# TJUMMG/OCPG

Hardware: AMD Instinct MI355X
Metric: clips/sec fwd+bwd (5x384x640, R101) (higher is better)
Workload: dtype bf16

## Files before the change

### include/ocpg_hip.h

```cpp
#ifndef OCPG_HIP_H
#define OCPG_HIP_H
#include <stdint.h>

#ifdef __cplusplus
extern "C" {
#endif

int ocpg_msda_fwd_f32(const float* value, const int64_t* shapes, const int64_t* level_start,
                      const float* loc, const float* attn,
                      int N, int S, int M, int D, int L, int Lq, int P,
                      float* out, const int64_t* shapes_host, void* stream);
int ocpg_msda_fwd_f64(const double* value, const int64_t* shapes, const int64_t* level_start,
                      const double* loc, const double* attn,
                      int N, int S, int M, int D, int L, int Lq, int P,
                      double* out, void* stream);

int ocpg_msda_bwd_f32(const float* value, const int64_t* shapes, const int64_t* level_start,
                      const float* loc, const float* attn, const float* grad_out,
                      int N, int S, int M, int D, int L, int Lq, int P,
                      float* grad_value, float* grad_loc, float* grad_attn,
                      const int64_t* shapes_host, void* stream);
int ocpg_msda_bwd_value_f32(const float* loc, const float* attn, const float* grad_out,
                            int N, int S, int M, int D, int L, int Lq, int P,
                            float* grad_value, const int64_t* shapes_host, void* stream);
// ... 11 lines not shown
                                  float* grad_qproj, void* stream);
int ocpg_msda_bwd_value_sel_f32(const float* loc, const float* attn, const float* grad_out,
                                int N, int S, int M, int D, int L, int Lq, int P,
                                float* grad_value, const int64_t* shapes_host, int* sel_state, void* stream);
int ocpg_msda_bwd_f64(const double* value, const int64_t* shapes, const int64_t* level_start,
                      const double* loc, const double* attn, const double* grad_out,
                      int N, int S, int M, int D, int L, int Lq, int P,
                      double* grad_value, double* grad_loc, double* grad_attn, void* stream);

int ocpg_msda_sf_fwd_f32(const float* src, const float* wv, const float* bv, const unsigned char* pad,
                         const int64_t* shapes, const int64_t* level_start, const float* loc, const float* attn,
                         int N, int S, int M, int D, int L, int Lq, int P,
                         float* out, float* s, float* beta, void* stream);
int ocpg_msda_sf_bwd_f32(const float* src, const float* wv, const float* bv, const unsigned char* pad,
                         const int64_t* shapes, const int64_t* level_start, const float* loc, const float* attn,
                         const float* grad_out, int N, int S, int M, int D, int L, int Lq, int P,
                         float* grad_src, float* grad_loc, float* grad_attn, void* stream);
int ocpg_msda_sf_bwd_params_f32(const float* grad_out, const float* s, const float* beta, int N, int M, int D, int Lq,
                                float* grad_wv, float* grad_bv, void* stream);

int ocpg_msda_fwd_h16(const void* value, const int64_t* shapes, const int64_t* level_start,
                      const float* loc, const float* attn,
                      int N, int S, int M, int D, int L, int Lq, int P,
                      void* out, const int64_t* shapes_host, int dtype, void* stream);
int ocpg_msda_bwd_h16(const void* value, const int64_t* shapes, const int64_t* level_start,
                      const float* loc, const float* attn, const void* grad_out,
                      int N, int S, int M, int D, int L, int Lq, int P,
                      float* grad_value, float* grad_loc, float* grad_attn,
                      const int64_t* shapes_host, int* sel_state, int dtype, void* stream);
int ocpg_msda_bwd_value_h16(const float* loc, const float* attn, const void* grad_out,
                            int N, int S, int M, int D, int L, int Lq, int P,
                            float* grad_value, const int64_t* shapes_host, int* sel_state, int dtype, void* stream);
int ocpg_msda_bwd_locattn_h16(const void* value, const int64_t* shapes, const int64_t* level_start,
                              const float* loc, const float* attn, const void* grad_out,
                              int N, int S, int M, int D, int L, int Lq, int P,
                              float* grad_loc, float* grad_attn, int dtype, void* stream);
int ocpg_msda_fused_fwd_h16(const void* value, const int64_t* shapes, const int64_t* level_start,
                            const float* qproj, const float* ref,
                            int N, int S, int M, int D, int L, int Lq, int P,
                            void* out, float* loc_out, float* attn_out, int dtype, void* stream);
int ocpg_msda_fused_bwd_qproj_h16(const void* value, const int64_t* shapes, const int64_t* level_start,
                                  const float* loc, const float* attn, const void* grad_out,
                                  int N, int S, int M, int D, int L, int Lq, int P,
                                  float* grad_qproj, int dtype, void* stream);

int ocpg_bn_act_fwd(const void* x, const float* scale, const float* shift, const void* skip, void* y,
                    long long n_outer, int C, long long inner, int relu, int dtype, void* stream);
int ocpg_bn_act_bwd(const void* gy, const void* y, const float* scale, void* gx, void* gskip,
                    long long n_outer, int C, long long inner, int relu, int dtype, void* stream);

int ocpg_gemm_dgrad_bn_tile(long long M, int N, int K);
int ocpg_gemm_dgrad_bn(const void* a, const void* w, const void* c, const void* mask, const float* scale, void* out, void* out_skip,
                       long long M, int N, int K, int dtype, int tile, void* stream);

int ocpg_win_attn_fwd(const void* qkv, const float* biasT, const int* region, float scale, int BW, int NW, int N, int H,
                      int head_dim, void* out, float* lse, int dtype, void* stream);
int ocpg_win_attn_bwd(const void* qkv, const float* bias, const float* biasT, const int* region, float scale, int BW, int NW,
                      int N, int H, int head_dim, const void* out, const void* dout, const float* lse, void* dqkv, float* Dbuf,
                      float* dbiasT, int dtype, void* stream);

int ocpg_win_attn_bwd_mfma(const void* qkv, const float* bias, const float* biasT, const int* region, float scale, int BW, int NW, int N,
                           int H, int head_dim, const void* out, const void* dout, const float* lse, void* dqkv, float* Dbuf, void* dS,
                           int dtype, void* stream);

int ocpg_win_attn_dtable_supported(int N, int head_dim, int dtype, int T);
int ocpg_win_attn_bwd_mfma_dtable(const void* qkv, const float* bias, const float* biasT, const int* region, float scale, int BW, int NW,
                                  int N, int H, int head_dim, const void* out, const void* dout, const float* lse, void* dqkv, float* Dbuf,
                                  const int* tok_code, int code_off, int T, float* partials, float* dtable, int dtype, void* stream);

int ocpg_dynmask_fwd_f32(const float* feats, const float* params, const float* refpix, int BT, int Q, int C, int H, int W,
                         int stride, float* out, float* pre1, void* stream);

int ocpg_dynmask_bwd_pre_f32(const float* dout, const float* pre1, const float* params, int BT, int Q, int C, int H, int W,
                             int stride, float* dpre, float* part, float* w0d, void* stream);
int ocpg_dynmask_bwd_fin_f32(const float* part, const float* params, const float* refpix, const float* dw0, int BT, int Q, int C,
                             int H, int W, float* dparams, float* dref, void* stream);

int ocpg_im2col3x3_nhwc(const void* x, int N, int H, int W, int C, int stride, int dil, void* cols, int dtype, void* stream);
int ocpg_col2im3x3_nhwc(const void* dcols, int N, int H, int W, int C, int stride, int dil, void* dx, int dtype, void* stream);

int ocpg_conv3x3_mfma_fwd(const void* x, const void* w, const float* scale, const float* bias, int relu, int N, int H, int W,
                          int Cin, int Cout, int stride, void* y, void* stream);
int ocpg_conv3x3_mfma_fwd_cols(const void* x, const void* w, const float* scale, const float* bias, int relu, int N, int H, int W, int Cin,
                               int Cout, int stride, void* y, void* cols, void* stream);
int ocpg_conv3x3_mfma_dgrad(const void* dy, const void* wT, int N, int H, int W, int Cin, int Cout, int stride, void* dx,
                            void* stream);
int ocpg_conv3x3_mfma_dgrad_masked(const void* dy, const void* wT, const void* mask_y, const float* scale, int N, int H, int W, int Cin,
                                   int Cout, int stride, void* dx, void* stream);
int ocpg_conv3x3_mfma_dgrad_w(const void* dy, const void* w, const void* mask_y, const float* scale, int N, int H, int W, int Cin, int Cout,
                              int stride, void* dx, void* stream);
int ocpg_conv3x3_mfma_body_splits(long long M, int ncols, int kchannels);
int ocpg_conv3x3_mfma_fwd_bn_splitk(const void* x, const void* w, const float* scale, const float* shift, int relu, int N, int H, int W, int Cin,
                                    int Cout, int stride, int splits, float* part, void* y, void* stream);
int ocpg_conv3x3_mfma_dgrad_w_splitk(const void* dy, const void* w, const void* mask_y, const float* scale, int N, int H, int W, int Cin,
                                     int Cout, int stride, int splits, float* part, void* dx, void* stream);
int ocpg_conv3x3_mfma_wgrad_splits(int N, int H, int W, int Cin, int Cout, int stride);
int ocpg_conv3x3_mfma_wgrad(const void* gz, const void* x, int N, int H, int W, int Cin, int Cout, int stride, void* part, void* stream);
int ocpg_conv3x3_mfma_fwd_cols_h16(const void* x, const void* w, const float* scale, const float* bias, int relu, int N, int H, int W, int Cin,
                                   int Cout, int stride, void* y, void* cols, int dtype, void* stream);
int ocpg_conv3x3_mfma_dgrad_w_h16(const void* dy, const void* w, const void* mask_y, const float* scale, int N, int H, int W, int Cin, int Cout,
                                  int stride, void* dx, int dtype, void* stream);
int ocpg_conv3x3_mfma_wgrad_h16(const void* gz, const void* x, int N, int H, int W, int Cin, int Cout, int stride, void* part, int dtype,
                                void* stream);
int ocpg_conv3x3_mfma_dgrad_w_s2(const void* dy, const void* w, const void* mask_y, const float* scale, int N, int H, int W, int Cin, int Cout,
                                 int stride, void* dx, void* stream);
int ocpg_conv3x3_mfma_dgrad_w_s2_h16(const void* dy, const void* w, const void* mask_y, const float* scale, int N, int H, int W, int Cin, int Cout,
// ... 201 lines not shown
```

### ocpg_amd/_lib.py

```python
import ctypes
import os

import torch

_HERE = os.path.dirname(os.path.abspath(__file__))
LIB_PATH = os.environ.get("OCPG_HIP_LIB") or os.path.join(_HERE, "lib", "libocpg_hip.so")
_lib = None

_i64p = ctypes.c_void_p
_vp = ctypes.c_void_p
_int = ctypes.c_int

SIGNATURES = {
    "ocpg_msda_fwd_f32": [_vp, _i64p, _i64p, _vp, _vp] + [_int] * 7 + [_vp, _vp, _vp],
    "ocpg_msda_fwd_f64": [_vp, _i64p, _i64p, _vp, _vp] + [_int] * 7 + [_vp, _vp],
    "ocpg_msda_bwd_f32": [_vp, _i64p, _i64p, _vp, _vp, _vp] + [_int] * 7 + [_vp, _vp, _vp, _vp, _vp],
    "ocpg_msda_bwd_value_f32": [_vp, _vp, _vp] + [_int] * 7 + [_vp, _vp, _vp],
    "ocpg_msda_fused_fwd_f32": [_vp, _i64p, _i64p, _vp, _vp] + [_int] * 7 + [_vp, _vp, _vp, _vp],
    "ocpg_msda_fused_bwd_qproj_f32": [_vp, _i64p, _i64p, _vp, _vp, _vp] + [_int] * 7 + [_vp, _vp],
    "ocpg_msda_bwd_value_sel_f32": [_vp, _vp, _vp] + [_int] * 7 + [_vp, _vp, _vp, _vp],
    "ocpg_msda_bwd_locattn_f32": [_vp, _i64p, _i64p, _vp, _vp, _vp] + [_int] * 7 + [_vp, _vp, _vp],
    "ocpg_msda_bwd_f64": [_vp, _i64p, _i64p, _vp, _vp, _vp] + [_int] * 7 + [_vp, _vp, _vp, _vp],
    "ocpg_msda_sf_fwd_f32": [_vp, _vp, _vp, _vp, _i64p, _i64p, _vp, _vp] + [_int] * 7 + [_vp, _vp, _vp, _vp],
    "ocpg_msda_sf_bwd_f32": [_vp, _vp, _vp, _vp, _i64p, _i64p, _vp, _vp, _vp] + [_int] * 7 + [_vp, _vp, _vp, _vp],
    "ocpg_msda_sf_bwd_params_f32": [_vp, _vp, _vp] + [_int] * 4 + [_vp, _vp, _vp],
    "ocpg_msda_fwd_h16": [_vp, _i64p, _i64p, _vp, _vp] + [_int] * 7 + [_vp, _vp, _int, _vp],
    "ocpg_msda_bwd_h16": [_vp, _i64p, _i64p, _vp, _vp, _vp] + [_int] * 7 + [_vp, _vp, _vp, _vp, _vp, _int, _vp],
    "ocpg_msda_bwd_value_h16": [_vp, _vp, _vp] + [_int] * 7 + [_vp, _vp, _vp, _int, _vp],
    "ocpg_msda_bwd_locattn_h16": [_vp, _i64p, _i64p, _vp, _vp, _vp] + [_int] * 7 + [_vp, _vp, _int, _vp],
    "ocpg_msda_fused_fwd_h16": [_vp, _i64p, _i64p, _vp, _vp] + [_int] * 7 + [_vp, _vp, _vp, _int, _vp],
    "ocpg_msda_fused_bwd_qproj_h16": [_vp, _i64p, _i64p, _vp, _vp, _vp] + [_int] * 7 + [_vp, _int, _vp],
    "ocpg_bn_act_fwd": [_vp, _vp, _vp, _vp, _vp, ctypes.c_longlong, _int, ctypes.c_longlong, _int, _int, _vp],
    "ocpg_bn_act_bwd": [_vp, _vp, _vp, _vp, _vp, ctypes.c_longlong, _int, ctypes.c_longlong, _int, _int, _vp],
    "ocpg_gemm_dgrad_bn_tile": [ctypes.c_longlong, _int, _int],
    "ocpg_gemm_dgrad_bn": [_vp] * 7 + [ctypes.c_longlong, _int, _int, _int, _int, _vp],
    "ocpg_dynmask_fwd_f32": [_vp, _vp, _vp] + [_int] * 6 + [_vp, _vp, _vp],
    "ocpg_dynmask_bwd_pre_f32": [_vp, _vp, _vp] + [_int] * 6 + [_vp, _vp, _vp, _vp],
    "ocpg_dynmask_bwd_fin_f32": [_vp, _vp, _vp, _vp] + [_int] * 5 + [_vp, _vp, _vp],
    "ocpg_conv3x3_mfma_fwd": [_vp, _vp, _vp, _vp] + [_int] * 7 + [_vp, _vp],
    "ocpg_conv3x3_mfma_fwd_cols": [_vp, _vp, _vp, _vp] + [_int] * 7 + [_vp, _vp, _vp],
    "ocpg_conv3x3_mfma_dgrad": [_vp, _vp] + [_int] * 6 + [_vp, _vp],
    "ocpg_conv3x3_mfma_dgrad_masked": [_vp, _vp, _vp, _vp] + [_int] * 6 + [_vp, _vp],
    "ocpg_conv3x3_mfma_dgrad_w": [_vp, _vp, _vp, _vp] + [_int] * 6 + [_vp, _vp],
    "ocpg_conv3x3_mfma_splits": [_int] * 6,
    "ocpg_conv3x3_mfma_wgrad_splits": [_int] * 6,
    "ocpg_conv3x3_mfma_body_splits": [ctypes.c_longlong, _int, _int],
    "ocpg_conv3x3_mfma_fwd_bn_splitk": [_vp, _vp, _vp, _vp] + [_int] * 8 + [_vp, _vp, _vp],
    "ocpg_conv3x3_mfma_dgrad_w_splitk": [_vp, _vp, _vp, _vp] + [_int] * 7 + [_vp, _vp, _vp],
    "ocpg_conv3x3_mfma_wgrad": [_vp, _vp] + [_int] * 6 + [_vp, _vp],
    "ocpg_conv3x3_mfma_fwd_cols_h16": [_vp, _vp, _vp, _vp] + [_int] * 7 + [_vp, _vp, _int, _vp],
    "ocpg_conv3x3_mfma_dgrad_w_h16": [_vp, _vp, _vp, _vp] + [_int] * 6 + [_vp, _int, _vp],
    "ocpg_conv3x3_mfma_wgrad_h16": [_vp, _vp] + [_int] * 6 + [_vp, _int, _vp],
    "ocpg_conv3x3_mfma_dgrad_w_s2": [_vp, _vp, _vp, _vp] + [_int] * 6 + [_vp, _vp],
    "ocpg_conv3x3_mfma_dgrad_w_s2_h16": [_vp, _vp, _vp, _vp] + [_int] * 6 + [_vp, _int, _vp],
    "ocpg_conv3x3_mfma_fwd_splitk": [_vp, _vp, _vp] + [_int] * 7 + [_vp, _vp, _int, _vp, _vp],
    "ocpg_conv3x3_mfma_fwd_splitk_h16": [_vp, _vp, _vp] + [_int] * 7 + [_vp, _vp, _int, _vp, _int, _vp],
    "ocpg_gemm": [_vp, _vp, _vp, _vp] + [_int] * 4 + [ctypes.c_longlong] * 10 + [ctypes.c_float, ctypes.c_float, _vp],
    "ocpg_gemm_plans": [],
    "ocpg_gemm_tuned": [_vp],
    "ocpg_gemm_tune_rejected": [],
    "ocpg_gemm_set_tuning": [_int],
    "ocpg_gemm_export_picks": [_vp, ctypes.c_longlong],
    "ocpg_gemm_import_picks": [_vp, ctypes.c_longlong],
    "ocpg_window_means3x3_fwd": [_vp, ctypes.c_longlong, _int, _int, _int, _vp, _vp],
    "ocpg_window_means3x3_bwd": [_vp, ctypes.c_longlong, _int, _int, _vp, _vp],
    "ocpg_window_sums3x3_cl_bands": [_int],
    "ocpg_window_sums3x3_cl": [_vp, _int, _int, _int, _int, _int, _vp, _vp],
    "ocpg_window_means3x3_bwd_cl": [_vp, _int, _int, _int, _int, _vp, _vp, _vp],
    "ocpg_mso_conv3x3": [_vp, _int, _int, _vp, _int, _vp, _vp, _int, _vp, _int, _vp, _vp, _int] + [_int] * 6 + [_vp],
    "ocpg_mso_wgrad_rows": [_int] * 4,
    "ocpg_mso_wgrad": [_vp, _int, _int, _vp, _vp, _vp] + [_int] * 8 + [_vp],
    "ocpg_bilinear_nhwc_fwd": [_vp] + [_int] * 6 + [_vp, _vp],
    "ocpg_bilinear_nhwc_bwd": [_vp] + [_int] * 6 + [_vp, _vp],
    "ocpg_small_linear_fwd": [_vp, _int, _vp, _vp, _int, _int, _int, _int, _vp, _vp],
    "ocpg_small_linear_bwd": [_vp, _int, _vp, _int, _vp, _vp, _int, _int, _int, _vp, _vp, _vp, _vp],
    "ocpg_small_linear_fwd_h16": [_vp, _int, _vp, _vp, _int, _int, _int, _int, _vp, _int, _vp],
    "ocpg_small_linear_bwd_h16": [_vp, _int, _vp, _int, _vp, _vp, _int, _int, _int, _vp, _vp, _vp, _int, _vp],
    "ocpg_small_linear_f32_fwd": [_vp, _vp, _vp, _int, _int, _int, _vp, _vp],
    "ocpg_small_linear_f32_bwd": [_vp, _vp, _vp, _int, _int, _int, _vp, _vp, _vp, _vp],
    "ocpg_layernorm_blocks": [ctypes.c_longlong],
    "ocpg_groupnorm_cl_work": [ctypes.c_longlong, _int, _int, _int],
    "ocpg_groupnorm_cl_fwd": [_vp, _int, _vp, _vp, ctypes.c_longlong, _int, _int, _int, ctypes.c_float, _vp, _vp, _vp, _vp, _vp],
    "ocpg_groupnorm_cl_bwd": [_vp, _vp, _int, _vp, _vp, _vp, ctypes.c_longlong, _int, _int, _int, _vp, _vp, _vp, _vp],
    "ocpg_groupnorm_cl2cl_fwd": [_vp, _int, _vp, _vp, ctypes.c_longlong, _int, _int, _int, ctypes.c_float, _vp, _vp, _vp, _vp, _vp],
    "ocpg_groupnorm_cl2cl_bwd": [_vp, _vp, _int, _vp, _vp, _vp, ctypes.c_longlong, _int, _int, _int, _vp, _vp, _vp, _vp],
    "ocpg_layernorm_fwd": [_vp, _int, _vp, _vp, ctypes.c_longlong, _int, ctypes.c_float, _vp, _int, _vp, _vp, _vp],
    "ocpg_layernorm_bwd": [_vp, _int, _vp, _int, _vp, _vp, _vp, ctypes.c_longlong, _int, _vp, _int, _vp, _vp, _vp],
    "ocpg_gather_rows_bwd": [_vp, _vp, _vp, _int, _int, _vp, _vp],
# ... 49 lines not shown
                                                             _vp, _vp, _int, _vp],
    "ocpg_attn_longk_fwd": [_vp, ctypes.c_longlong, _vp, ctypes.c_longlong, _vp, ctypes.c_longlong, _vp, ctypes.c_float] + [_int] * 5
                           + [ctypes.c_float, ctypes.c_ulonglong, ctypes.c_ulonglong, _vp, _vp, ctypes.c_longlong, _vp, _int, _vp],
    "ocpg_attn_longk_bwd": [_vp, ctypes.c_longlong, _vp, ctypes.c_longlong, _vp, ctypes.c_longlong, _vp, _vp, ctypes.c_longlong, _vp,
                            ctypes.c_longlong, _vp, ctypes.c_float] + [_int] * 5 + [ctypes.c_float, ctypes.c_ulonglong, ctypes.c_ulonglong, _vp,
                                                                                    _vp, ctypes.c_longlong, _vp, _vp, _int, _vp],
    "ocpg_text_gate_rows": [_int],
    "ocpg_text_gate_splits": [_int],
    "ocpg_text_gate_fwd_h16": [_vp] * 6 + [ctypes.c_float] + [_int] * 5 + [_vp, _int, _vp],
    "ocpg_text_gate_bwd_h16": [_vp] * 7 + [ctypes.c_float] + [_int] * 5 + [_vp, _vp, _vp, _int, _vp],
    "ocpg_mask_tail_f32": [_vp] + [_int] * 10 + [ctypes.c_float, ctypes.c_float, _int, _vp, _vp],
    "ocpg_jf_counts_u8": [_vp, _vp] + [_int] * 8 + [_vp, _vp],
    "ocpg_refmask_counts_f32": [_vp] + [_int] * 5 + [_vp] * 4 + [_int, _int, ctypes.c_float, _int, _vp, _vp],
    "ocpg_sim_heat_workspace": [_int] * 4,
    "ocpg_sim_heat_f32": [_vp] + [_int] * 5 + [_vp] * 10,
    "ocpg_win_attn_fwd": [_vp, _vp, _vp, ctypes.c_float] + [_int] * 5 + [_vp, _vp, _int, _vp],
    "ocpg_win_attn_bwd": [_vp, _vp, _vp, _vp, ctypes.c_float] + [_int] * 5 + [_vp] * 6 + [_int, _vp],
    "ocpg_win_attn_bwd_mfma": [_vp, _vp, _vp, _vp, ctypes.c_float] + [_int] * 5 + [_vp] * 6 + [_int, _vp],
    "ocpg_win_attn_dtable_supported": [_int] * 4,
    "ocpg_win_attn_bwd_mfma_dtable": [_vp, _vp, _vp, _vp, ctypes.c_float] + [_int] * 5 + [_vp] * 6 + [_int, _int, _vp, _vp, _int, _vp],
}


_TIMING = {"on": False, "events": []}
_UNTIMED = ("ocpg_sim_heat_workspace", "ocpg_text_gate_rows", "ocpg_text_gate_splits", "ocpg_win_attn_dtable_supported", "ocpg_conv3x3_mfma_body_splits", "ocpg_gemm_dgrad_bn_tile", "ocpg_conv3x3_mfma_wgrad_splits", "ocpg_window_sums3x3_cl_bands", "ocpg_lfm_dft_supported", "ocpg_lfm_dft_split", "ocpg_conv3x3_mfma_splits", "ocpg_gemm_set_tuning", "ocpg_gemm_export_picks", "ocpg_gemm_import_picks", "ocpg_colsum_blocks", "ocpg_mso_wgrad_rows", "ocpg_gemm_plans", "ocpg_gemm_tuned", "ocpg_gemm_tune_rejected", "ocpg_bias_relu_dropout_bwd_slots", "ocpg_dropout_add_ln_bwd_slots", "ocpg_groupnorm_cl_work")


def enable_kernel_timing(on=True):
    _TIMING["on"] = on
    _TIMING["events"] = []


def collect_kernel_timing(work=None):
    torch.cuda.synchronize()
    out = {}
    for name, args, e0, e1 in _TIMING["events"]:
        d = out.setdefault(name, {"ms": 0.0, "n": 0, "work": 0.0, "modelled": 0})
        d["ms"] += e0.elapsed_time(e1)
        d["n"] += 1
        w = work(name, args) if work is not None else None
        if isinstance(w, tuple):
            d["work_lowp"] = d.get("work_lowp", 0.0) + (w[0] if w[1] else 0.0)
            w = w[0]
        if w is not None:
            d["work"] += w
            d["modelled"] += 1
    _TIMING["events"] = []
    _TIMING["on"] = False
    return out


CENSUS = {"on": False, "calls": {}}
CENSUS_ALSO = {"ocpg_conv3x3_mfma_dgrad_w_s2": "ocpg_conv3x3_mfma_dgrad_w", "ocpg_conv3x3_mfma_dgrad_w_s2_h16": "ocpg_conv3x3_mfma_dgrad_w_h16",
               "ocpg_dropout_add_ln_fwd_ex": "ocpg_dropout_add_ln_fwd", "ocpg_dropout_add_ln_bwd_ex": "ocpg_dropout_add_ln_bwd"}


def census(on=True):
    CENSUS["on"] = on
    if on:
        CENSUS["calls"] = {}
    return CENSUS["calls"]


class _Lib:

    def __init__(self, cdll):
        self._cdll = cdll

    def __getattr__(self, name):
        fn = getattr(self._cdll, name)
        if name not in SIGNATURES or name in _UNTIMED:
            setattr(self, name, fn)
            return fn
        timed = not name.startswith("ocpg_msda_")

        def call(*a):
            if CENSUS["on"]:
                rc = fn(*a)
                if rc == 0:
                    for k in (name, CENSUS_ALSO.get(name)):
                        if k is not None:
                            CENSUS["calls"][k] = CENSUS["calls"].get(k, 0) + 1
                return rc
            if not (timed and _TIMING["on"]):
                return fn(*a)
            e0, e1 = torch.cuda.Event(enable_timing=True), torch.cuda.Event(enable_timing=True)
            e0.record()
            rc = fn(*a)
            e1.record()
            _TIMING["events"].append((name, tuple(getattr(x, "value", x) for x in a), e0, e1))
            return rc
        setattr(self, name, call)
        return call


def lib():
    global _lib
    if _lib is None:
        if not os.path.exists(LIB_PATH):
            raise RuntimeError(
                f"{LIB_PATH} not found: build it with `python -m ocpg_amd.csrc.build` "
                "(hipcc --offload-arch=gfx950). The HIP extension is mandatory; there is no CPU/PyTorch fallback.")
        L = ctypes.CDLL(LIB_PATH)
        for name, argtypes in SIGNATURES.items():
            fn = getattr(L, name)
            fn.argtypes = argtypes
            fn.restype = ctypes.c_int
# ... 32 lines not shown
```

### ocpg_amd/csrc/gemm_dgrad_bn.hip

```cpp
#include <hip/hip_bf16.h>
#include <hip/hip_fp16.h>
#include <hip/hip_runtime.h>
#include <stdint.h>

#include "../../include/ocpg_hip.h"
#include "h16_elem.h"

namespace {

typedef ocpg_h16::h16x8 bf16x8;
typedef short s4 __attribute__((ext_vector_type(4)));
typedef ocpg_h16::f32x16 f32x16;
typedef unsigned u32x4 __attribute__((ext_vector_type(4)));

constexpr int BK = 64, NT = 256;
constexpr int ALD = BK + 8;

constexpr int DECLINE_SHAPE = -2000, DECLINE_ALIGN = -2001, DECLINE_DTYPE = -2002;

struct Bf16 : ocpg_h16::Bf16 {
  static __device__ __forceinline__ void unpack8(const uint4 u, float (&f)[8]) {
    const uint32_t w[4] = {u.x, u.y, u.z, u.w};
#pragma unroll
    for (int i = 0; i < 4; ++i) {
// ... 15 lines not shown
#pragma unroll
    for (int i = 0; i < 4; ++i) {
      const float2 t = __half22float2(h[i]);
      f[2 * i] = t.x;
      f[2 * i + 1] = t.y;
    }
  }
  static __device__ __forceinline__ uint4 pack8(const float (&f)[8]) {
    uint32_t w[4];
#pragma unroll
    for (int i = 0; i < 4; ++i)
      w[i] = (uint32_t)__half_as_ushort(__float2half_rn(f[2 * i])) | ((uint32_t)__half_as_ushort(__float2half_rn(f[2 * i + 1])) << 16);
    return make_uint4(w[0], w[1], w[2], w[3]);
  }
};

template <typename T>
struct EpiT {
  const T* c;
  const T* mask;
  const float* scale;
  T* out;
  T* out_skip;
};
using Epi = EpiT<__hip_bfloat16>;

struct In8 { uint4 c, y; };
template <typename T>
__device__ __forceinline__ In8 load8(const EpiT<T>& e, long long off) {
  In8 r{make_uint4(0u, 0u, 0u, 0u), make_uint4(0u, 0u, 0u, 0u)};
  if (e.c) r.c = *reinterpret_cast<const uint4*>(e.c + off);
  if (e.mask) r.y = *reinterpret_cast<const uint4*>(e.mask + off);
  return r;
}

template <typename E>
__device__ __forceinline__ void epilogue8(const EpiT<typename E::T>& e, long long off, int col, float (&v)[8], const In8& in) {
  if (e.c) {
    float c[8];
    E::unpack8(in.c, c);
#pragma unroll
    for (int i = 0; i < 8; ++i) v[i] += c[i];
  }
  if (e.mask) {
    float y[8];
    E::unpack8(in.y, y);
#pragma unroll
    for (int i = 0; i < 8; ++i) v[i] = y[i] > 0.f ? v[i] : 0.f;
  }
  if (e.out_skip) *reinterpret_cast<uint4*>(e.out_skip + off) = E::pack8(v);
  if (e.scale) {
    const float4 s0 = reinterpret_cast<const float4*>(e.scale + col)[0], s1 = reinterpret_cast<const float4*>(e.scale + col)[1];
    v[0] *= s0.x, v[1] *= s0.y, v[2] *= s0.z, v[3] *= s0.w, v[4] *= s1.x, v[5] *= s1.y, v[6] *= s1.z, v[7] *= s1.w;
  }
  *reinterpret_cast<uint4*>(e.out + off) = E::pack8(v);
}

template <typename E, int TM, int TN>
__device__ __forceinline__ void gemm_dgrad_bn_body(const typename E::T* __restrict__ a, const typename E::T* __restrict__ w,
                                                   const EpiT<typename E::T>& e, long long M, int N, int K, int mtiles, int ntiles) {
  using T = typename E::T;
  constexpr int BLD = TN + 8;
  constexpr int SLD = TN + 4;
  constexpr int WM = TM / 2, WN = TN / 2, IM = WM / 32, JN = WN / 32;
  constexpr int A_L = TM * BK / 8 / NT;
  constexpr int BSEG = TN / 8, BROWS = NT / BSEG, B_L = BK / BROWS;
  constexpr int SMEM_SHORTS = 2 * (TM * ALD + BK * BLD);
  static_assert(TM * SLD * 2 <= SMEM_SHORTS, "the fp32 tile fits the staging buffers");
  __shared__ __attribute__((aligned(16))) short smem[SMEM_SHORTS];
  short (*As)[TM * ALD] = reinterpret_cast<short (*)[TM * ALD]>(smem);
  short (*Bs)[BK * BLD] = reinterpret_cast<short (*)[BK * BLD]>(smem + 2 * TM * ALD);
  const int tid = threadIdx.x, lane = tid & 63, wave = tid >> 6;
  const int wm = wave & 1, wn = wave >> 1;
  const unsigned total = gridDim.x;
  unsigned t = blockIdx.x;
  if ((total & 7u) == 0) t = (t & 7u) * (total >> 3) + (t >> 3);
  const long long m0 = (long long)(t / ntiles) * TM;
  const int n0 = (int)(t % ntiles) * TN;
  const int ksteps = K / BK;

  const int arow = tid >> 3, aseg = tid & 7, kr = tid / BSEG, bseg = tid % BSEG;
  const T* ap[A_L];
#pragma unroll
  for (int i = 0; i < A_L; ++i) {
    const long long r = min(m0 + arow + 32 * i, M - 1);
    ap[i] = a + r * K + aseg * 8;
  }
  const T* wp = w + (long long)kr * N + n0 + bseg * 8;
  const long long wstep = (long long)BROWS * N;

  auto fetch = [&](u32x4 (&Ra)[A_L], u32x4 (&Rb)[B_L], int s) __attribute__((always_inline)) {
    const int ks = min(s, ksteps - 1);
#pragma unroll
    for (int i = 0; i < A_L; ++i) Ra[i] = *reinterpret_cast<const u32x4*>(ap[i] + ks * BK);
    const T* wk = wp + (long long)ks * BK * N;
#pragma unroll
    for (int i = 0; i < B_L; ++i) Rb[i] = *reinterpret_cast<const u32x4*>(wk + i * wstep);
  };
  auto park = [&](int buf, const u32x4 (&Ra)[A_L], const u32x4 (&Rb)[B_L]) __attribute__((always_inline)) {
#pragma unroll
    for (int i = 0; i < A_L; ++i) *reinterpret_cast<u32x4*>(&As[buf][(arow + 32 * i) * ALD + aseg * 8]) = Ra[i];
#pragma unroll
    for (int i = 0; i < B_L; ++i) *reinterpret_cast<u32x4*>(&Bs[buf][(kr + BROWS * i) * BLD + bseg * 8]) = Rb[i];
  };

  f32x16 acc[IM * JN];
// ... 33 lines not shown
  park(0, R0a, R0b);
  __syncthreads();
  for (int s = 0; s < ksteps; s += 2) {
    fetch(R0a, R0b, s + 2);
    compute(0);
    park(1, R1a, R1b);
    __syncthreads();
    fetch(R1a, R1b, s + 3);
    compute(1);
    park(0, R0a, R0b);
    __syncthreads();
  }

  float* st = reinterpret_cast<float*>(smem);
  float* st0 = st + (wm * WM + 4 * fh) * SLD + wn * WN + fr;
#pragma unroll
  for (int r = 0; r < 16; ++r) {
    float* p = st0 + ((r & 3) + 8 * (r >> 2)) * SLD;
#pragma unroll
    for (int i = 0; i < IM; ++i)
#pragma unroll
      for (int j = 0; j < JN; ++j) p[i * 32 * SLD + j * 32] = acc[i * JN + j][r];
  }
  __syncthreads();
  constexpr int NQ = TM * TN / 8 / NT;
  In8 in[NQ];
#pragma unroll
  for (int q = 0; q < NQ; ++q) {
    const int idx = tid + q * NT;
    const long long grow = m0 + idx / BSEG;
    in[q] = grow < M ? load8(e, grow * N + n0 + (idx % BSEG) * 8) : In8{make_uint4(0u, 0u, 0u, 0u), make_uint4(0u, 0u, 0u, 0u)};
  }
#pragma unroll
  for (int q = 0; q < NQ; ++q) {
    const int idx = tid + q * NT, row = idx / BSEG, c8 = (idx % BSEG) * 8;
    const long long grow = m0 + row;
    if (grow >= M) continue;
    const float4 x0 = *reinterpret_cast<const float4*>(&st[row * SLD + c8]), x1 = *reinterpret_cast<const float4*>(&st[row * SLD + c8 + 4]);
    float v[8] = {x0.x, x0.y, x0.z, x0.w, x1.x, x1.y, x1.z, x1.w};
    epilogue8<E>(e, grow * N + n0 + c8, n0 + c8, v, in[q]);
  }
}

template <int TM, int TN>
__global__ __launch_bounds__(NT) void gemm_dgrad_bn(const __hip_bfloat16* __restrict__ a, const __hip_bfloat16* __restrict__ w, Epi e,
                                                    long long M, int N, int K, int mtiles, int ntiles) {
  gemm_dgrad_bn_body<Bf16, TM, TN>(a, w, e, M, N, K, mtiles, ntiles);
}

template <int TM, int TN>
__global__ __launch_bounds__(NT) void gemm_dgrad_bn_f16(const __half* __restrict__ a, const __half* __restrict__ w, EpiT<__half> e,
                                                        long long M, int N, int K, int mtiles, int ntiles) {
  gemm_dgrad_bn_body<Fp16, TM, TN>(a, w, e, M, N, K, mtiles, ntiles);
}

constexpr int TILE_M[3] = {128, 64, 64}, TILE_N[3] = {128, 128, 64};

inline bool aligned16(const void* p) { return ((uintptr_t)p & 15u) == 0; }

}

extern "C" int ocpg_gemm_dgrad_bn_tile(long long M, int N, int K) {
  if (M <= 0 || N <= 0 || K <= 0 || N % TILE_N[2] != 0 || K % (2 * BK) != 0) return -1;
  return 2;
}

extern "C" int ocpg_gemm_dgrad_bn(const void* a, const void* w, const void* c, const void* mask, const float* scale, void* out, void* out_skip,
                                  long long M, int N, int K, int dtype, int tile, void* stream) {
  if (dtype != 1 && dtype != 2) return DECLINE_DTYPE;
  if (M < 0 || N <= 0 || K <= 0) return -1007;
  if (tile < 0 || tile > 2) return -1011;
  if (N % TILE_N[tile] != 0 || K % (2 * BK) != 0) return DECLINE_SHAPE;
  if (!a) return -1001;
  if (!w) return -1002;
  if (!out) return -1006;
  const void* ptrs[] = {a, w, c, mask, scale, out, out_skip};
  for (const void* p : ptrs)
    if (p && !aligned16(p)) return DECLINE_ALIGN;
  if (M == 0) return 0;
  const hipStream_t st = (hipStream_t)stream;
  const int mtiles = (int)((M + TILE_M[tile] - 1) / TILE_M[tile]), ntiles = N / TILE_N[tile];
  const dim3 grid((unsigned)(mtiles * ntiles)), block(NT);
  if (dtype == 2) {
    const EpiT<__half> e{(const __half*)c, (const __half*)mask, scale, (__half*)out, (__half*)out_skip};
    const __half *ap = (const __half*)a, *wp = (const __half*)w;
    if (tile == 0) gemm_dgrad_bn_f16<128, 128><<<grid, block, 0, st>>>(ap, wp, e, M, N, K, mtiles, ntiles);
    else if (tile == 1) gemm_dgrad_bn_f16<64, 128><<<grid, block, 0, st>>>(ap, wp, e, M, N, K, mtiles, ntiles);
    else gemm_dgrad_bn_f16<64, 64><<<grid, block, 0, st>>>(ap, wp, e, M, N, K, mtiles, ntiles);
    const hipError_t err = hipGetLastError();
    return err == hipSuccess ? 0 : -(int)err;
  }
  const Epi e{(const __hip_bfloat16*)c, (const __hip_bfloat16*)mask, scale, (__hip_bfloat16*)out, (__hip_bfloat16*)out_skip};
  const __hip_bfloat16 *ap = (const __hip_bfloat16*)a, *wp = (const __hip_bfloat16*)w;
  if (tile == 0) gemm_dgrad_bn<128, 128><<<grid, block, 0, st>>>(ap, wp, e, M, N, K, mtiles, ntiles);
  else if (tile == 1) gemm_dgrad_bn<64, 128><<<grid, block, 0, st>>>(ap, wp, e, M, N, K, mtiles, ntiles);
  else gemm_dgrad_bn<64, 64><<<grid, block, 0, st>>>(ap, wp, e, M, N, K, mtiles, ntiles);
  const hipError_t err = hipGetLastError();
  return err == hipSuccess ? 0 : -(int)err;
}
```

### ocpg_amd/models/ops/functions/conv_bn_func.py

```python
import os

import torch
from torch.autograd import Function
from torch.autograd.function import once_differentiable

from ...._lib import check, lib

_DT = {torch.float32: 0, torch.bfloat16: 1, torch.float16: 2}
_H16 = (torch.bfloat16, torch.float16)
_CL = torch.channels_last
EPILOGUE = os.environ.get("OCPG_GEMM_EPILOGUE", "1") != "0"
FWD_COLS = os.environ.get("OCPG_CONV3X3_FWD_COLS", "0") != "0"
SKIP_GRAD_IN_GEMM = os.environ.get("OCPG_SKIP_GRAD_IN_GEMM", "1") != "0"
_SKIP_TOKENS = {}
PREMASK = os.environ.get("OCPG_PREMASK_DGRAD", "1") != "0"
_PREMASK_TOKENS = {}
FUSED_DGRAD_BN = os.environ.get("OCPG_FUSED_DGRAD_BN", "1") != "0"
_DGRAD_BN_DECLINED = (-2000, -2001, -2002)


def reset_skip_tokens():
    _SKIP_TOKENS.clear()
    _PREMASK_TOKENS.clear()


def _same_tensor(a, b):
    if a is None or b is None:
        return False
    return a is b or (a.data_ptr() == b.data_ptr() and a.shape == b.shape and a.dtype == b.dtype and a.stride() == b.stride()
                      and a._version == b._version)


def _tensor_key(t):
    return (t.data_ptr(), tuple(t.shape), t.dtype, tuple(t.stride()), t._version)


def _both16(*ts):
    return ts[0].dtype in _H16 and all(t.dtype == ts[0].dtype for t in ts)


def _offer_token(y, scale, skip, switch):
    tok = {"y": _tensor_key(y), "scale": scale, "skip": skip, "switch": switch, "gz": None, "gskip": None, "ver": None}
    _PREMASK_TOKENS[y.data_ptr()] = tok
    return tok


def _claim_token(x):
    tok = _PREMASK_TOKENS.pop(x.data_ptr(), None)
    return tok if (tok is not None and tok["y"] == _tensor_key(x)) else None


def _fill_token(tok, gz, gskip=None):
    tok["gz"], tok["gskip"], tok["ver"] = gz, gskip, gz._version


def _take_token(tok, gy):
    if tok is None or tok["gz"] is None:
        return None
    gz, gskip, ver = tok["gz"], tok["gskip"], tok["ver"]
    tok["gz"] = tok["gskip"] = tok["ver"] = None
    if not (gy.data_ptr() == gz.data_ptr() and gy.shape == gz.shape and gy.stride() == gz.stride() and gy._version == ver):
        raise RuntimeError(f"{tok['switch']}=1: the gradient of this conv + BN + ReLU output was produced with the BN + ReLU backward already "
                           f"applied by its consumer's input-gradient kernel, but a different gradient arrived (a second consumer of the "
                           f"output, or a gradient hook); run with {tok['switch']}=0 for such a graph")
    return gz, gskip


def _dgrad_bn(a, w, c, mask, scale, out, out_skip, m, n, k, st):
    L = lib()
    tile = int(L.ocpg_gemm_dgrad_bn_tile(m, n, k))
    if tile < 0:
        return _DGRAD_BN_DECLINED[0]
    rc = L.ocpg_gemm_dgrad_bn(a.data_ptr(), w.data_ptr(), None if c is None else c.data_ptr(), mask.data_ptr(), scale.data_ptr(), out.data_ptr(),
                              None if out_skip is None else out_skip.data_ptr(), m, n, k, _DT.get(a.dtype, -1), tile, st)
    if rc and rc not in _DGRAD_BN_DECLINED:
        check(rc, "ocpg_gemm_dgrad_bn")
    return rc


def _reduce_partials(part, w_is_cast_copy):
    from ... import amp_cache
    if w_is_cast_copy and amp_cache.DEFER_SUM and amp_cache.MULTI_CAST and part.dtype in (torch.bfloat16, torch.float16):
        return amp_cache.defer_sum(part)
    return part.sum(0)


def eligible(x, conv):
    return (x.is_cuda and x.dim() == 4 and x.dtype in _DT and conv.kernel_size == (1, 1) and conv.stride == (1, 1) and conv.padding == (0, 0)
            and conv.groups == 1 and conv.bias is None and x.is_contiguous(memory_format=_CL))


def eligible_s2(x, conv):
    return (x.is_cuda and x.dim() == 4 and x.dtype in _DT and conv.kernel_size == (1, 1) and conv.stride == (2, 2) and conv.padding == (0, 0)
            and conv.groups == 1 and conv.bias is None and x.is_contiguous(memory_format=_CL))


class Subsample2(Function):

    @staticmethod
    def forward(ctx, x):
        ctx.shape = x.shape
        return x[:, :, ::2, ::2].contiguous(memory_format=_CL)

    @staticmethod
    @once_differentiable
    def backward(ctx, g):
        gx = torch.empty(ctx.shape, dtype=g.dtype, device=g.device, memory_format=_CL).zero_()
        gx[:, :, ::2, ::2] = g
        return gx


def subsample2(x):
    return Subsample2.apply(x)


class Conv1x1BNAct(Function):
    @staticmethod
    def forward(ctx, x, w, scale, shift, skip, relu, splits):
        n, c, h, wd = x.shape
        co = w.shape[0]
        m = n * h * wd
        dt = _DT[x.dtype]
# ... 418 lines not shown
```

Baseline: 63.64.

## Add persistent software-pipelined dgrad+BN GEMM kernel with prefetched epilogue inputs

Adds a persistent 64x64-tile GEMM kernel for the fused dgrad + BN/ReLU epilogue. Each workgroup loops over several output tiles in a grid-stride schedule, double-buffers the K loop through registers and shared memory, and prefetches the next tile's A/W fragments and epilogue inputs (skip, mask, scale) while it computes and writes the current tile. The grid is capped at three workgroups per CU with a fixed occupancy hint, and the kernel is enabled by default in place of the tile-selected launch. The aim is to hide global-load latency and launch tail effects, at the cost of more register pressure and a single fixed tile shape that may be worse for large GEMMs than the old 128x128 tile.

```diff
diff --git a/include/ocpg_hip.h b/include/ocpg_hip.h
--- a/include/ocpg_hip.h
+++ b/include/ocpg_hip.h
@@ -87,6 +87,8 @@
 int ocpg_gemm_dgrad_bn_tile(long long M, int N, int K);
 int ocpg_gemm_dgrad_bn(const void* a, const void* w, const void* c, const void* mask, const float* scale, void* out, void* out_skip,
                        long long M, int N, int K, int dtype, int tile, void* stream);
+int ocpg_gemm_dgrad_bn_pipe(const void* a, const void* w, const void* c, const void* mask, const float* scale, void* out, void* out_skip,
+                            long long M, int N, int K, int dtype, int wgs, int ksplit, void* stream);
 
 int ocpg_win_attn_fwd(const void* qkv, const float* biasT, const int* region, float scale, int BW, int NW, int N, int H,
                       int head_dim, void* out, float* lse, int dtype, void* stream);
diff --git a/ocpg_amd/_lib.py b/ocpg_amd/_lib.py
--- a/ocpg_amd/_lib.py
+++ b/ocpg_amd/_lib.py
@@ -34,6 +34,7 @@
     "ocpg_bn_act_bwd": [_vp, _vp, _vp, _vp, _vp, ctypes.c_longlong, _int, ctypes.c_longlong, _int, _int, _vp],
     "ocpg_gemm_dgrad_bn_tile": [ctypes.c_longlong, _int, _int],
     "ocpg_gemm_dgrad_bn": [_vp] * 7 + [ctypes.c_longlong, _int, _int, _int, _int, _vp],
+    "ocpg_gemm_dgrad_bn_pipe": [_vp] * 7 + [ctypes.c_longlong, _int, _int, _int, _int, _int, _vp],
     "ocpg_dynmask_fwd_f32": [_vp, _vp, _vp] + [_int] * 6 + [_vp, _vp, _vp],
     "ocpg_dynmask_bwd_pre_f32": [_vp, _vp, _vp] + [_int] * 6 + [_vp, _vp, _vp, _vp],
     "ocpg_dynmask_bwd_fin_f32": [_vp, _vp, _vp, _vp] + [_int] * 5 + [_vp, _vp, _vp],
@@ -189,7 +190,8 @@
 
 CENSUS = {"on": False, "calls": {}}
 CENSUS_ALSO = {"ocpg_conv3x3_mfma_dgrad_w_s2": "ocpg_conv3x3_mfma_dgrad_w", "ocpg_conv3x3_mfma_dgrad_w_s2_h16": "ocpg_conv3x3_mfma_dgrad_w_h16",
-               "ocpg_dropout_add_ln_fwd_ex": "ocpg_dropout_add_ln_fwd", "ocpg_dropout_add_ln_bwd_ex": "ocpg_dropout_add_ln_bwd"}
+               "ocpg_dropout_add_ln_fwd_ex": "ocpg_dropout_add_ln_fwd", "ocpg_dropout_add_ln_bwd_ex": "ocpg_dropout_add_ln_bwd",
+               "ocpg_gemm_dgrad_bn_pipe": "ocpg_gemm_dgrad_bn"}
 
 
 def census(on=True):
diff --git a/ocpg_amd/csrc/gemm_dgrad_bn.hip b/ocpg_amd/csrc/gemm_dgrad_bn.hip
--- a/ocpg_amd/csrc/gemm_dgrad_bn.hip
+++ b/ocpg_amd/csrc/gemm_dgrad_bn.hip
@@ -91,6 +91,28 @@
   if (e.scale) {
     const float4 s0 = reinterpret_cast<const float4*>(e.scale + col)[0], s1 = reinterpret_cast<const float4*>(e.scale + col)[1];
     v[0] *= s0.x, v[1] *= s0.y, v[2] *= s0.z, v[3] *= s0.w, v[4] *= s1.x, v[5] *= s1.y, v[6] *= s1.z, v[7] *= s1.w;
+  }
+  *reinterpret_cast<uint4*>(e.out + off) = E::pack8(v);
+}
+
+template <typename E>
+__device__ __forceinline__ void epilogue8_pre(const EpiT<typename E::T>& e, long long off, float (&v)[8], const In8& in, const float (&s)[8]) {
+  if (e.c) {
+    float c[8];
+    E::unpack8(in.c, c);
+#pragma unroll
+    for (int i = 0; i < 8; ++i) v[i] += c[i];
+  }
+  if (e.mask) {
+    float y[8];
+    E::unpack8(in.y, y);
+#pragma unroll
+    for (int i = 0; i < 8; ++i) v[i] = y[i] > 0.f ? v[i] : 0.f;
+  }
+  if (e.out_skip) *reinterpret_cast<uint4*>(e.out_skip + off) = E::pack8(v);
+  if (e.scale) {
+#pragma unroll
+    for (int i = 0; i < 8; ++i) v[i] *= s[i];
   }
   *reinterpret_cast<uint4*>(e.out + off) = E::pack8(v);
 }
@@ -230,6 +252,158 @@
 __global__ __launch_bounds__(NT) void gemm_dgrad_bn_f16(const __half* __restrict__ a, const __half* __restrict__ w, EpiT<__half> e,
                                                         long long M, int N, int K, int mtiles, int ntiles) {
   gemm_dgrad_bn_body<Fp16, TM, TN>(a, w, e, M, N, K, mtiles, ntiles);
+}
+
+template <typename E>
+__device__ __forceinline__ void gemm_dgrad_bn_pipe_body(const typename E::T* __restrict__ a, const typename E::T* __restrict__ w,
+                                                        const EpiT<typename E::T>& e, long long M, int N, int K, unsigned total, int ntiles) {
+  using T = typename E::T;
+  constexpr int TM = 64, TN = 64;
+  constexpr int D = 2;
+  constexpr int BLD = TN + 8, SLD = TN + 4;
+  constexpr int A_L = TM * BK / 8 / NT;
+  constexpr int BSEG = TN / 8, BROWS = NT / BSEG, B_L = BK / BROWS;
+  constexpr int BUF = TM * ALD + BK * BLD;
+  static_assert(TM * SLD * 2 <= BUF, "the fp32 tile fits one staging buffer");
+  __shared__ __attribute__((aligned(16))) short smem[2 * BUF];
+  const int tid = threadIdx.x, lane = tid & 63, wave = tid >> 6;
+  const int wm = wave & 1, wn = wave >> 1;
+  const int ksteps = K / BK;
+
+  unsigned t = blockIdx.x, tstride = gridDim.x, tend = total;
+  if ((gridDim.x & 7u) == 0) {
+    const unsigned per = (total + 7u) >> 3, x = blockIdx.x & 7u;
+    t = x * per + (blockIdx.x >> 3);
+    tstride = gridDim.x >> 3;
+    tend = min(total, (x + 1u) * per);
+  }
+  if (t >= tend) return;
+
+  const int arow = tid >> 3, aseg = tid & 7, kr = tid / BSEG, bseg = tid % BSEG;
+  const T* ap[A_L];
+  const T* wp;
+  const long long wstep = (long long)BROWS * N;
+  auto aim = [&](unsigned tt, long long& tm0, int& tn0) __attribute__((always_inline)) {
+    tm0 = (long long)(tt / (unsigned)ntiles) * TM;
+    tn0 = (int)(tt % (unsigned)ntiles) * TN;
+#pragma unroll
+    for (int i = 0; i < A_L; ++i) ap[i] = a + min(tm0 + arow + 32 * i, M - 1) * K + aseg * 8;
+    wp = w + (long long)kr * N + tn0 + bseg * 8;
+  };
+  auto fetch = [&](u32x4 (&Ra)[A_L], u32x4 (&Rb)[B_L], int ks) __attribute__((always_inline)) {
+#pragma unroll
+    for (int i = 0; i < A_L; ++i) Ra[i] = *reinterpret_cast<const u32x4*>(ap[i] + ks * BK);
+    const T* wk = wp + (long long)ks * BK * N;
+#pragma unroll
+    for (int i = 0; i < B_L; ++i) Rb[i] = *reinterpret_cast<const u32x4*>(wk + i * wstep);
+  };
+  auto park = [&](int buf, const u32x4 (&Ra)[A_L], const u32x4 (&Rb)[B_L]) __attribute__((always_inline)) {
+    short* As = smem + buf * BUF;
+    short* Bs = As + TM * ALD;
+#pragma unroll
+    for (int i = 0; i < A_L; ++i) *reinterpret_cast<u32x4*>(&As[(arow + 32 * i) * ALD + aseg * 8]) = Ra[i];
+#pragma unroll
+    for (int i = 0; i < B_L; ++i) *reinterpret_cast<u32x4*>(&Bs[(kr + BROWS * i) * BLD + bseg * 8]) = Rb[i];
+  };
+
+  f32x16 acc;
+  const int fr = lane & 31, fh = lane >> 5;
+  auto compute = [&](int buf) __attribute__((always_inline)) {
+    const short* As = smem + buf * BUF;
+    const short* Bs = As + TM * ALD;
+    const int li = lane & 15, grp = lane >> 4;
+#pragma unroll
+    for (int kk = 0; kk < BK / 16; ++kk) {
+      const bf16x8 af = *reinterpret_cast<const bf16x8*>(&As[(wm * 32 + fr) * ALD + kk * 16 + fh * 8]);
+      const short* p = &Bs[(kk * 16 + 8 * fh + (li >> 2)) * BLD + wn * 32 + 16 * (grp & 1) + 4 * (li & 3)];
+      const s4 lo = __builtin_amdgcn_ds_read_tr16_b64_v4i16((__attribute__((address_space(3))) s4*)p);
+      const s4 hi = __builtin_amdgcn_ds_read_tr16_b64_v4i16((__attribute__((address_space(3))) s4*)(p + 4 * BLD));
+      bf16x8 bf;
+      bf[0] = lo[0]; bf[1] = lo[1]; bf[2] = lo[2]; bf[3] = lo[3]; bf[4] = hi[0]; bf[5] = hi[1]; bf[6] = hi[2]; bf[7] = hi[3];
+      acc = E::mfma(af, bf, acc);
+    }
+  };
+
+  constexpr int NQ = TM * TN / 8 / NT;
+  In8 in[NQ];
+  auto load_in = [&](int q, long long tm0, int tn0) __attribute__((always_inline)) {
+    const int idx = tid + q * NT;
+    const long long grow = tm0 + idx / BSEG;
+    in[q] = grow < M ? load8(e, grow * N + tn0 + (idx % BSEG) * 8) : In8{make_uint4(0u, 0u, 0u, 0u), make_uint4(0u, 0u, 0u, 0u)};
+  };
+  static_assert(NT % BSEG == 0, "a thread's NQ segments are the same 8 columns");
+  float sc[8] = {1.f, 1.f, 1.f, 1.f, 1.f, 1.f, 1.f, 1.f};
+  auto load_scale = [&](int tn0) __attribute__((always_inline)) {
+    if (!e.scale) return;
+    const float4* p = reinterpret_cast<const float4*>(e.scale + tn0 + (tid % BSEG) * 8);
+    const float4 s0 = p[0], s1 = p[1];
+    sc[0] = s0.x, sc[1] = s0.y, sc[2] = s0.z, sc[3] = s0.w, sc[4] = s1.x, sc[5] = s1.y, sc[6] = s1.z, sc[7] = s1.w;
+  };
+
+  long long m0;
+  int n0;
+  u32x4 Ra[D][A_L], Rb[D][B_L];
+  aim(t, m0, n0);
+#pragma unroll
+  for (int j = 0; j < D; ++j) fetch(Ra[j], Rb[j], j);
+#pragma unroll
+  for (int q = 0; q < NQ; ++q) load_in(q, m0, n0);
+  load_scale(n0);
+  park(0, Ra[0], Rb[0]);
+  __syncthreads();
+  float* st = reinterpret_cast<float*>(smem + BUF);
+  for (;;) {
+#pragma unroll
+    for (int r = 0; r < 16; ++r) acc[r] = 0.f;
+    const unsigned tnext = t + tstride;
+    const bool more = tnext < tend;
+    long long nm0 = m0;
+    int nn0 = n0;
+    int s = 0;
+    do {
+      int ks = s + D;
+      if (ks == ksteps) {
+        if (more) aim(tnext, nm0, nn0);
+        ks = 0;
+      }
+#pragma unroll
+      for (int j = 0; j < D; ++j) {
+        fetch(Ra[j], Rb[j], ks + j);
+        compute(j & 1);
+        park((j + 1) & 1, Ra[(j + 1) % D], Rb[(j + 1) % D]);
+        __syncthreads();
+      }
+    } while ((s += D) < ksteps);
+    float* st0 = st + (wm * 32 + 4 * fh) * SLD + wn * 32 + fr;
+#pragma unroll
+    for (int r = 0; r < 16; ++r) st0[((r & 3) + 8 * (r >> 2)) * SLD] = acc[r];
+    __syncthreads();
+#pragma unroll
+    for (int q = 0; q < NQ; ++q) {
+      const int idx = tid + q * NT, row = idx / BSEG, c8 = (idx % BSEG) * 8;
+      const long long grow = m0 + row;
+      if (grow < M) {
+        const float4 x0 = *reinterpret_cast<const float4*>(&st[row * SLD + c8]), x1 = *reinterpret_cast<const float4*>(&st[row * SLD + c8 + 4]);
+        float v[8] = {x0.x, x0.y, x0.z, x0.w, x1.x, x1.y, x1.z, x1.w};
+        epilogue8_pre<E>(e, grow * N + n0 + c8, v, in[q], sc);
+      }
+      if (more) load_in(q, nm0, nn0);
+    }
+    if (!more) break;
+    load_scale(nn0);
+    t = tnext, m0 = nm0, n0 = nn0;
+    __syncthreads();
+  }
+}
+
+__global__ __launch_bounds__(NT) __attribute__((amdgpu_waves_per_eu(4, 4))) void gemm_dgrad_bn_pipe(const __hip_bfloat16* __restrict__ a, const __hip_bfloat16* __restrict__ w, Epi e,
+                                                         long long M, int N, int K, unsigned total, int ntiles) {
+  gemm_dgrad_bn_pipe_body<Bf16>(a, w, e, M, N, K, total, ntiles);
+}
+
+__global__ __launch_bounds__(NT) __attribute__((amdgpu_waves_per_eu(4, 4))) void gemm_dgrad_bn_pipe_f16(const __half* __restrict__ a, const __half* __restrict__ w, EpiT<__half> e,
+                                                             long long M, int N, int K, unsigned total, int ntiles) {
+  gemm_dgrad_bn_pipe_body<Fp16>(a, w, e, M, N, K, total, ntiles);
 }
 
 constexpr int TILE_M[3] = {128, 64, 64}, TILE_N[3] = {128, 128, 64};
@@ -276,3 +450,44 @@
   const hipError_t err = hipGetLastError();
   return err == hipSuccess ? 0 : -(int)err;
 }
+
+static unsigned pipe_workgroups(unsigned tiles) {
+  static int cus = 0;
+  if (cus == 0) {
+    int dev = 0, n = 0;
+    if (hipGetDevice(&dev) != hipSuccess || hipDeviceGetAttribute(&n, hipDeviceAttributeMultiprocessorCount, dev) != hipSuccess || n <= 0) n = 256;
+    cus = n;
+  }
+  const unsigned slots = 3u * (unsigned)cus;
+  return tiles < slots ? tiles : slots;
+}
+
+extern "C" int ocpg_gemm_dgrad_bn_pipe(const void* a, const void* w, const void* c, const void* mask, const float* scale, void* out,
+                                       void* out_skip, long long M, int N, int K, int dtype, int wgs, int ksplit, void* stream) {
+  if (dtype != 1 && dtype != 2) return DECLINE_DTYPE;
+  if (M < 0 || N <= 0 || K <= 0) return -1007;
+  if (wgs < 0 || ksplit < 0 || ksplit > 1) return -1011;
+  if (N % TILE_N[2] != 0 || K % (2 * BK) != 0) return DECLINE_SHAPE;
+  if (!a) return -1001;
+  if (!w) return -1002;
+  if (!out) return -1006;
+  const void* ptrs[] = {a, w, c, mask, scale, out, out_skip};
+  for (const void* p : ptrs)
+    if (p && !aligned16(p)) return DECLINE_ALIGN;
+  if (M == 0) return 0;
+  const int ntiles = N / TILE_N[2];
+  const long long tiles = (M + TILE_M[2] - 1) / TILE_M[2] * ntiles;
+  if (tiles > 0x7fffffffLL) return -1007;
+  const unsigned total = (unsigned)tiles;
+  const dim3 grid(wgs > 0 ? ((unsigned)wgs < total ? (unsigned)wgs : total) : pipe_workgroups(total)), block(NT);
+  const hipStream_t st = (hipStream_t)stream;
+  if (dtype == 2) {
+    const EpiT<__half> e{(const __half*)c, (const __half*)mask, scale, (__half*)out, (__half*)out_skip};
+    gemm_dgrad_bn_pipe_f16<<<grid, block, 0, st>>>((const __half*)a, (const __half*)w, e, M, N, K, total, ntiles);
+  } else {
+    const Epi e{(const __hip_bfloat16*)c, (const __hip_bfloat16*)mask, scale, (__hip_bfloat16*)out, (__hip_bfloat16*)out_skip};
+    gemm_dgrad_bn_pipe<<<grid, block, 0, st>>>((const __hip_bfloat16*)a, (const __hip_bfloat16*)w, e, M, N, K, total, ntiles);
+  }
+  const hipError_t err = hipGetLastError();
+  return err == hipSuccess ? 0 : -(int)err;
+}
diff --git a/ocpg_amd/models/ops/functions/conv_bn_func.py b/ocpg_amd/models/ops/functions/conv_bn_func.py
--- a/ocpg_amd/models/ops/functions/conv_bn_func.py
+++ b/ocpg_amd/models/ops/functions/conv_bn_func.py
@@ -16,6 +16,7 @@
 PREMASK = os.environ.get("OCPG_PREMASK_DGRAD", "1") != "0"
 _PREMASK_TOKENS = {}
 FUSED_DGRAD_BN = os.environ.get("OCPG_FUSED_DGRAD_BN", "1") != "0"
+DGRAD_BN_PIPE = os.environ.get("OCPG_DGRAD_BN_PIPE", "1") != "0"
 _DGRAD_BN_DECLINED = (-2000, -2001, -2002)
 
 
@@ -68,6 +69,12 @@
 
 def _dgrad_bn(a, w, c, mask, scale, out, out_skip, m, n, k, st):
     L = lib()
+    if DGRAD_BN_PIPE:
+        rc = L.ocpg_gemm_dgrad_bn_pipe(a.data_ptr(), w.data_ptr(), None if c is None else c.data_ptr(), mask.data_ptr(), scale.data_ptr(),
+                                       out.data_ptr(), None if out_skip is None else out_skip.data_ptr(), m, n, k, _DT.get(a.dtype, -1), 0, 0, st)
+        if rc and rc not in _DGRAD_BN_DECLINED:
+            check(rc, "ocpg_gemm_dgrad_bn_pipe")
+        return rc
     tile = int(L.ocpg_gemm_dgrad_bn_tile(m, n, k))
     if tile < 0:
         return _DGRAD_BN_DECLINED[0]
```

Measured after the change: 63.90 (median of 6 runs). No clear change (+0.4%).
